# JihyongOh/DeMFI

Hardware: AMD Instinct MI355X
Metric: interpolated frames/sec @720p x8 MFI (N_tst=3) (higher is better)
Workload: dtype f16; 1 GPU; DeMFI-Net_rb N_tst=3, x8 MFI, 720x1280 (padded 736x1280), fp16, clip-parallel windows, random-init weights; uint8 frames host->HBM->host inside the timed region (PNG codec excluded), 8 distinct windows; graph=True, parallelism=clip1, n_ctx=7, n_trunk=3

## Files before the change

### demfi_amd/csrc/conv_wstream.hip

```cpp
#include "conv_common.h"

namespace {

#ifndef DEMFI_WS3_DEPTH
#define DEMFI_WS3_DEPTH 9
#endif
#ifndef DEMFI_WS_NW
#define DEMFI_WS_NW 4
#endif
template <int KS, int NW, int NCH = 2, int TH_ = 16> struct WsCfg {
    static constexpr int TH = TH_;
    static constexpr int RPW = TH / (NW / NCH);
    static constexpr int BL = KS + RPW - 1;
    static constexpr int LH = TH + KS - 1;
    static constexpr int LL = KS == 7 ? ((TW + KS - 1 + 7) & ~7) : TW + KS - 1;
    static constexpr int NI = (LH * LL + 15) / 16;
    static constexpr int UNIT_BYTES = NI * 1024;
    static constexpr int LDS_BYTES = 2 * UNIT_BYTES;
    static constexpr int NG = 2 * KS;
    static constexpr int NSTEP = NG * KS;
    static constexpr int DEPTH = NW == 8 ? KS : (KS == 7 ? 2 * KS : DEMFI_WS3_DEPTH);
    static constexpr int NIW = (NI + NW - 1) / NW;
    static constexpr int DMA_EVERY = KS == 7 ? 6 : 1;
    static constexpr int DMA_PER = KS == 7 ? 1 : 3;
    static constexpr bool PIECE_STRIDES = KS != 7;
    static_assert(LDS_BYTES <= 160 * 1024, "two units must fit LDS");
    static_assert((NIW + DMA_PER - 1) / DMA_PER * DMA_EVERY + DEPTH <= NSTEP, "the unit's DMA must be older than the last A fragment consumed in the unit");
    static_assert(NSTEP % DEPTH == 0, "static ring indices");
};

template <int KS, int NW, int NCH = 2, int TH_ = 16>
__global__ __launch_bounds__(64 * NW, 1) void conv_wstream_c64_kernel(const demfi_conv* __restrict__ d)
{
    using C = WsCfg<KS, NW, NCH, TH_>;
    constexpr int WS_TH = C::TH;
    constexpr int RPW = C::RPW;
    extern __shared__ __attribute__((aligned(16))) char smem[];
    const int tid = threadIdx.x;
    const int lane = tid & 63;
    const int wave = __builtin_amdgcn_readfirstlane(tid >> 6);
    const int hi = lane >> 5, lx = lane & 31;
    const int cs = NCH == 2 ? (wave & 1) : 0, rh = NCH == 2 ? (wave >> 1) : wave;
    const int H = d->H, W = d->W;
    const int tiles_x = (W + TW - 1) / TW, tiles_y = (H + WS_TH - 1) / WS_TH, tiles_img = tiles_x * tiles_y;
    const int total = tiles_img * d->batch;
    int t_first, t_end, t_step;
    {
        const int G = gridDim.x;
        if ((G & 7) == 0 && total >= G) {
            const int xcd = blockIdx.x & 7, idx = blockIdx.x >> 3;
            const int q = (total + 7) >> 3, lo = xcd * q;
            t_first = lo + idx;
            t_end = min(lo + q, total);
            t_step = G >> 3;
        } else {
            t_first = blockIdx.x;
            t_end = total;
            t_step = G;
        }
    }
    if (t_first >= t_end) return;
    const int upt = d->n_chunks;
    const int n_units = ((t_end - t_first + t_step - 1) / t_step) * upt;

    const demfi_piece& p0 = d->pieces[d->chunks[0].first_piece];
    const int64_t sxb = p0.v.sx * 2, syb = p0.v.sy * 2, sbb = p0.v.sb * 2;
    const char* const zeros = (const char*)d->zero_page;
    const uint4* const wbase = (const uint4*)d->wpack;

    int doff[C::NIW], dlc[C::NIW];
#pragma unroll
    for (int j = 0; j < C::NIW; ++j) {
        const int rec = min((wave + NW * j) * 16 + (lane >> 2), C::LH * C::LL - 1);
        const int l = rec / C::LL, c = rec - l * C::LL;
        doff[j] = C::PIECE_STRIDES ? (((lane & 3) ^ ((c >> 2) & 3)) << 4) : (int)(l * syb + c * sxb) + (((lane & 3) ^ ((c >> 2) & 3)) << 4);
        dlc[j] = l | (c << 8);
    }
    int boff[C::NG];
#pragma unroll
    for (int g = 0; g < C::NG; ++g) {
        const int col = lx + (g >> 1);
        boff[g] = (rh * RPW * C::LL + col) * 64 + ((((g & 1) * 2 + hi) ^ ((col >> 2) & 3)) << 4);
    }

    struct Unit { const char* src; const char* w; int iy0, ix0; bool interior; int sx, sy; };
    const unsigned lane16 = lane * 16;
    auto unit_info = [&](int u) {
        Unit r;
        const int k = u / upt, cu = u - k * upt;
        const int it = t_first + k * t_step;
        const int bimg = it / tiles_img, rem = it - bimg * tiles_img;
        const int ty = rem / tiles_x, tx = rem - ty * tiles_x;
        r.iy0 = ty * WS_TH - KS / 2;
        r.ix0 = tx * TW - KS / 2;
        const demfi_piece& pc = d->pieces[d->chunks[cu].first_piece];
        r.sx = C::PIECE_STRIDES ? (int)(pc.v.sx * 2) : (int)sxb;
        r.sy = C::PIECE_STRIDES ? (int)(pc.v.sy * 2) : (int)syb;
        r.src = (const char*)pc.v.ptr + bimg * (C::PIECE_STRIDES ? pc.v.sb * 2 : sbb) + (int64_t)r.iy0 * r.sy + (int64_t)r.ix0 * r.sx;
        r.w = (const char*)(wbase + d->chunks[cu].w_off + cs * 64);
        r.interior = r.iy0 >= 0 && r.iy0 + C::LH <= H && r.ix0 >= 0 && r.ix0 + C::LL <= W;
        return r;
    };
    auto dma_one = [&](auto J, const Unit& un, char* buf) {
        constexpr int j = decltype(J)::value;
        const int i = wave + NW * j;
        if (i >= C::NI) return;
        const char* g = un.src + doff[j];
        if constexpr (C::PIECE_STRIDES) g += (dlc[j] & 255) * un.sy + (dlc[j] >> 8) * un.sx;
        if (!un.interior) {
            const int iy = un.iy0 + (dlc[j] & 255), ix = un.ix0 + (dlc[j] >> 8);
            if (!(iy >= 0 && iy < H && ix >= 0 && ix < W)) g = zeros;
        }
        const unsigned la = (unsigned)(uintptr_t)(__attribute__((address_space(3))) char*)(buf + i * 1024);
#if defined(__HIP_DEVICE_COMPILE__)
        unsigned m0_save;
        asm volatile("s_mov_b32 %0, m0\n\ts_mov_b32 m0, %2\n\ts_nop 0\n\tglobal_load_lds_dwordx4 %1, off\n\ts_mov_b32 m0, %0"
                     : "=&s"(m0_save) : "v"(g), "s"(la) : "memory");
#endif
    };
    auto a_load = [&](const Unit& un, int t) {
        const int g = t / KS, ky = t - g * KS, kx = g >> 1, ksl = g & 1;
        return __builtin_bit_cast(uint4, *gcp<u4_t>(un.w + (unsigned)((((ky * KS + kx) * 2 + ksl) * NCH) * 1024 + lane16)));
    };

    const demfi_seg& sg = d->segs[d->sub_seg[0]];
    half_t* const dstp = (half_t*)sg.dst.ptr;
    const int act = sg.act;
    const int ch0 = d->oct_ch[0];
    f4_t bq[4];
#pragma unroll
    for (int qd = 0; qd < 4; ++qd) bq[qd] = *gcp<f4_t>(d->bias + cs * 32 + qd * 8 + hi * 4);

    f16x_t acc[RPW];
#pragma unroll
    for (int p = 0; p < RPW; ++p) {
#pragma unroll
        for (int i = 0; i < 16; ++i) acc[p][i] = 0.0f;
    }
    uint4 A[C::DEPTH];
    Unit cur = unit_info(0);
    static_for<0, C::NIW>([&](auto J) { dma_one(J, cur, smem); });
    static_for<0, C::DEPTH>([&](auto T) { A[decltype(T)::value] = a_load(cur, decltype(T)::value); });
    asm volatile("s_waitcnt vmcnt(%0)" ::"n"(C::DEPTH) : "memory");
    asm volatile("s_barrier" ::: "memory");

    for (int u = 0; u < n_units; ++u) {
        const bool has_next = u + 1 < n_units;
        TRACE_STAMP(wave, u / upt, u % upt);
        const Unit nxt = unit_info(has_next ? u + 1 : 0);
        const char* const tb = smem + (u & 1) * C::UNIT_BYTES;
        char* const nb = smem + ((u + 1) & 1) * C::UNIT_BYTES;
        uint4 B[2][C::BL];
#pragma unroll
        for (int r = 0; r < RPW; ++r) B[0][r] = *(const uint4*)(tb + boff[0] + r * (C::LL * 64));
        __builtin_amdgcn_sched_barrier(0);
        static_for<0, C::NSTEP>([&](auto T_) {
            constexpr int t = decltype(T_)::value;
            constexpr int g = t / KS, ky = t % KS, gb = g & 1;
            const uint4 a = A[t % C::DEPTH];
            if constexpr (ky + RPW < C::BL) B[gb][ky + RPW] = *(const uint4*)(tb + boff[g] + (ky + RPW) * (C::LL * 64));
            if constexpr (g + 1 < C::NG) {
                if constexpr (ky < RPW) B[gb ^ 1][ky] = *(const uint4*)(tb + boff[g + 1] + ky * (C::LL * 64));
                if constexpr (ky == KS - 1) {
#pragma unroll
                    for (int r = KS; r < RPW; ++r) B[gb ^ 1][r] = *(const uint4*)(tb + boff[g + 1] + r * (C::LL * 64));
                }
            }
            if constexpr (t + C::DEPTH < C::NSTEP) A[t % C::DEPTH] = a_load(cur, t + C::DEPTH);
            else                                   A[t % C::DEPTH] = a_load(nxt, t + C::DEPTH - C::NSTEP);
            if constexpr (KS == 7) {
                if constexpr (t % C::DMA_EVERY == 2 && t / C::DMA_EVERY < C::NIW) {
                    if (has_next) dma_one(std::integral_constant<int, t / C::DMA_EVERY>{}, nxt, nb);
                }
            } else {
                if (has_next) {
                    static_for<0, C::DMA_PER>([&](auto Q) {
                        constexpr int j = t * C::DMA_PER + decltype(Q)::value;
                        if constexpr (j < C::NIW) dma_one(std::integral_constant<int, j>{}, nxt, nb);
                    });
                }
            }
#pragma unroll
            for (int p = 0; p < RPW; ++p) Mma<half_t>::run(acc[p], a, B[gb][ky + p]);
            __builtin_amdgcn_sched_barrier(0);
        });
        asm volatile("s_waitcnt vmcnt(%0)" ::"n"(C::DEPTH) : "memory");
        const int k = u / upt;
        if (u - k * upt == upt - 1) {
            const int it = t_first + k * t_step;
            const int bimg = it / tiles_img, rem = it - bimg * tiles_img;
            const int ty = rem / tiles_x, tx = rem - ty * tiles_x;
            const int ox = tx * TW + lx;
#pragma unroll
            for (int p = 0; p < RPW; ++p) {
                const int oy = ty * WS_TH + rh * RPW + p;
#pragma unroll
                for (int m2 = 0; m2 < 2; ++m2) {
                    float v[8];
#pragma unroll
                    for (int j = 0; j < 4; ++j) {
                        v[j] = acc[p][(2 * m2) * 4 + j] + bq[2 * m2][j];
                        v[4 + j] = acc[p][(2 * m2 + 1) * 4 + j] + bq[2 * m2 + 1][j];
                    }
                    apply_act_n<8>(v, act);
                    if (oy < H && ox < W)
                        store8<half_t>(dstp + bimg * sg.dst.sb + oy * sg.dst.sy + ox * sg.dst.sx + ch0 + cs * 32 + m2 * 16 + hi * 8, v);
                }
#pragma unroll
                for (int i = 0; i < 16; ++i) acc[p][i] = 0.0f;
            }
        }
        asm volatile("s_barrier" ::: "memory");
        cur = nxt;
    }
}

static bool wstream_eligible(const demfi_conv* h, int ks = 7, int nch = 2)
{
    if (h->dtype != DEMFI_F16 || h->stride != 1 || h->kh != ks || h->kw != ks || h->pad_y != ks / 2 || h->pad_x != ks / 2) return false;
    if (h->inH != h->H || h->inW != h->W || !h->zero_page || h->rec_bytes != 64) return false;
    if (h->n_chunks < (ks == 7 ? 1 : 2) || h->cout_pad != 32 * nch || h->nco != nch) return false;
    const demfi_piece& p0 = h->pieces[h->chunks[0].first_piece];
    for (int c = 0; c < h->n_chunks; ++c) {
        const demfi_chunk& ch = h->chunks[c];
        if (ch.n_pieces != 1 || ch.nks != 2) return false;
        const demfi_piece& p = h->pieces[ch.first_piece];
        if (!p.fat || p.nch != 32 || p.up_shift || !p.v.ptr || p.v.sc != 1 || p.v.is_f32) return false;
        if (ks == 7 && (p.v.sx != p0.v.sx || p.v.sy != p0.v.sy || p.v.sb != p0.v.sb)) return false;
        if (p.v.sy < 0 || p.v.sx < 0 || p.v.sy >= (int64_t)1 << 31 || p.v.sx >= (int64_t)1 << 31) return false;
        if (p.v.sy * 2 * 40 + p.v.sx * 2 * 48 >= (int64_t)1 << 31) return false;
    }
    const int sgi = h->sub_seg[0];
    if (sgi < 0 || (nch == 2 && (h->sub_seg[1] != sgi || h->oct_ch[4] != h->oct_ch[0] + 32))) return false;
    for (int o = 0; o < 4 * nch; ++o)
        if (h->oct_seg[o] != sgi || h->oct_n[o] != 8 || h->oct_ch[o] != h->oct_ch[0] + 8 * o) return false;
    const demfi_seg& sg = h->segs[sgi];
    if (sg.mode != DEMFI_MODE_STORE || sg.scale != 1 || sg.dy || sg.dx || sg.res.ptr || !sg.dst.ptr || sg.dst.is_f32 || sg.dst.sc != 1) return false;
    return true;
}

static int launch_wstream3(const demfi_conv* h, const demfi_conv* dev, hipStream_t st)
{
    DEMFI_LDS_ATTR((conv_wstream_c64_kernel<3, 4, 1, 32>));
    const int total = ((h->W + TW - 1) / TW) * ((h->H + 31) / 32) * h->batch;
    const int grid = total >= 256 ? 256 : total;
    constexpr size_t lds = WsCfg<3, 4, 1, 32>::LDS_BYTES;
    hipLaunchKernelGGL((conv_wstream_c64_kernel<3, 4, 1, 32>), dim3(grid), dim3(256), lds, st, dev);
    DEMFI_HIP_CHECK(hipGetLastError());
    return DEMFI_OK;
}

static int launch_wstream(const demfi_conv* h, const demfi_conv* dev, hipStream_t st)
{
    DEMFI_LDS_ATTR((conv_wstream_c64_kernel<7, DEMFI_WS_NW>));
    const int total = ((h->W + TW - 1) / TW) * ((h->H + 15) / 16) * h->batch;
    const int grid = total >= 256 ? 256 : total;
    constexpr size_t lds = WsCfg<7, DEMFI_WS_NW>::LDS_BYTES;
    hipLaunchKernelGGL((conv_wstream_c64_kernel<7, DEMFI_WS_NW>), dim3(grid), dim3(64 * DEMFI_WS_NW), lds, st, dev);
    DEMFI_HIP_CHECK(hipGetLastError());
    return DEMFI_OK;
}


}

int demfi_wstream_trace_collect(unsigned long long* acc) { return TRACE_DRAIN(acc, true); }

bool demfi_wstream_eligible(const demfi_conv* h, int ks, int nch) { return wstream_eligible(h, ks, nch); }
int demfi_wstream_launch(const demfi_conv* h, const demfi_conv* dev, hipStream_t st) { return launch_wstream(h, dev, st); }
int demfi_wstream3_launch(const demfi_conv* h, const demfi_conv* dev, hipStream_t st) { return launch_wstream3(h, dev, st); }
```

### demfi_amd/csrc/gru.hip

```cpp
#include "kernel_kit.h"
#include <cstdlib>

namespace {

constexpr int G_LS = 32 * 128;
constexpr int G_NH = 4;
constexpr int G_NTHREADS = 256 + 64 * G_NH;
#ifndef DEMFI_GRU_DEPTH
#define DEMFI_GRU_DEPTH 4
#endif
constexpr int G_DEPTH = DEMFI_GRU_DEPTH;
constexpr int G_NSTEP = 20;
static_assert(G_NSTEP % G_DEPTH == 0, "static ring indices");
enum { GM_R = 1, GM_ZQS = 2 };
template <int MODE> struct GCfg;
template <> struct GCfg<GM_R>   { static constexpr int TL = 16, WL = 20, NPIECE = 2, LDS = 2 * 20 * G_LS; };
template <> struct GCfg<GM_ZQS> { static constexpr int TL = 8, WL = 12, NPIECE = 3, LDS = 3 * 12 * G_LS + 512; };
static_assert(GCfg<GM_R>::LDS <= 160 * 1024 && GCfg<GM_ZQS>::LDS <= 160 * 1024, "LDS budget");
constexpr int ZS_D = 8;
constexpr int ZS_NA = 80;
static_assert(ZS_NA % ZS_D == 0, "static ring indices");

DEMFI_TRACE_BUFFER(32, 8, 24, 10)

// ... 4 lines not shown
    asm("v_fma_mix_f32 %0, -%1, %2, %3 op_sel_hi:[1,0,0]" : "=v"(d) : "v"(h), "v"(b), "v"(c));
#endif
    return d;
}
__device__ __forceinline__ float g_nfma_hi(float b, unsigned h, float c)
{
    float d = 0.0f;
#if defined(__HIP_DEVICE_COMPILE__)
    asm("v_fma_mix_f32 %0, -%1, %2, %3 op_sel:[1,0,0] op_sel_hi:[1,0,0]" : "=v"(d) : "v"(h), "v"(b), "v"(c));
#endif
    return d;
}

__device__ __forceinline__ float g_sub16_lo(unsigned q, unsigned h)
{
    float d = 0.0f;
#if defined(__HIP_DEVICE_COMPILE__)
    asm("v_fma_mix_f32 %0, %1, -1.0, %2 op_sel_hi:[1,0,1]" : "=v"(d) : "v"(h), "v"(q));
#endif
    return d;
}
__device__ __forceinline__ float g_sub16_hi(unsigned q, unsigned h)
{
    float d = 0.0f;
#if defined(__HIP_DEVICE_COMPILE__)
    asm("v_fma_mix_f32 %0, %1, -1.0, %2 op_sel:[1,0,1] op_sel_hi:[1,0,1]" : "=v"(d) : "v"(h), "v"(q));
#endif
    return d;
}
__device__ __forceinline__ void g_fma16_lo(unsigned& pk, float a, float b, unsigned c)
{
#if defined(__HIP_DEVICE_COMPILE__)
    asm("v_fma_mixlo_f16 %0, %1, %2, %3 op_sel_hi:[0,0,1]" : "+v"(pk) : "v"(a), "v"(b), "v"(c));
#endif
}
__device__ __forceinline__ void g_fma16_hi(unsigned& pk, float a, float b, unsigned c)
{
#if defined(__HIP_DEVICE_COMPILE__)
    asm("v_fma_mixhi_f16 %0, %1, %2, %3 op_sel:[0,0,1] op_sel_hi:[0,0,1]" : "+v"(pk) : "v"(a), "v"(b), "v"(c));
#endif
}

struct GPiece { const char* ptr; int64_t sl, sp, sb; };
struct GArgs {
    GPiece h, rh, x;
    char* dst; int64_t d_sl, d_sp, d_sb;
    const char* w0[2];
    const char* w1[2];
    const float* b0; const float* b1;
    const char* zeros;
    int Llen, Plen, batch, n_pt, n_ls;
};

template <int MODE>
__global__ __launch_bounds__(G_NTHREADS, 1) void gru_sep5_kernel(const GArgs a)
{
    using Cfg = GCfg<MODE>;
    constexpr int TL = Cfg::TL, WL = Cfg::WL, PIECE = WL * G_LS;
    constexpr int NI = WL * 4, NIW = NI / G_NH;
    static_assert(NIW == WL, "helper dw owns pixels 8 dw .. 8 dw + 7 of every line");
    extern __shared__ __attribute__((aligned(16))) char smem[];
    const int tid = threadIdx.x;
    const int lane = tid & 63;
    const int wave = __builtin_amdgcn_readfirstlane(tid >> 6);
    const int per_img = a.n_pt * a.n_ls;
    const int total = per_img * a.batch;
    int it0, it1;
    XCD_ITEM_RUN(total, it0, it1);
    if (it0 >= it1) return;
    auto pos_of = [&](int it, int& img, int& P0, int& L0) {
        img = it / per_img;
        const int rem = it - img * per_img;
        const int pt = rem / a.n_ls;
        P0 = pt * 32;
        L0 = (rem - pt * a.n_ls) * TL;
    };
    char* const S0 = smem;
    char* const S1 = smem + PIECE;
    char* const S2 = smem + 2 * PIECE;

    if constexpr (MODE == GM_ZQS) {
        if (tid < 128) ((float*)(smem + 3 * PIECE))[tid] = tid < 64 ? a.b0[tid] : a.b1[tid - 64];
        asm volatile("s_waitcnt lgkmcnt(0)" ::: "memory");
    }
    if (wave >= 4) {
        const int dw = wave - 4;
        __builtin_assume(dw >= 0 && dw < G_NH);
        const int px = dw * 8 + (lane >> 3);
        const unsigned slot16 = (unsigned)(((lane & 7) ^ ((px >> 1) & 7)) << 4);
        auto issue_piece = [&](const GPiece& pc, char* lds, int img, int P0, int L0, bool carry) {
            const char* base = pc.ptr + (int64_t)img * pc.sb + (int64_t)(L0 - 2) * pc.sl + (int64_t)P0 * pc.sp;
            const unsigned voff = (unsigned)(px * pc.sp) + slot16;
            const bool pok = P0 + px < a.Plen;
            u4_t halo[4];
            if (carry) {
#pragma unroll
                for (int j = 0; j < 4; ++j) halo[j] = *(const u4_t*)(lds + (4 * (TL + j) + dw) * 1024 + lane * 16);
                asm volatile("s_waitcnt lgkmcnt(0)" ::: "memory");
            }
            if (L0 - 2 >= 0 && L0 - 2 + WL <= a.Llen && P0 + 32 <= a.Plen) {
#pragma unroll
                for (int k = 0; k < NIW; ++k) {
                    if (k < 4 && carry) continue;
                    const char* lb = base + (int64_t)k * pc.sl;
                    lb = (const char*)(((uint64_t)(unsigned)__builtin_amdgcn_readfirstlane((int)((uint64_t)lb >> 32)) << 32) |
                                       (uint64_t)(unsigned)__builtin_amdgcn_readfirstlane((int)(uint64_t)lb));
                    unsigned v = voff;
                    asm volatile("" : "+v"(v));
                    __builtin_amdgcn_global_load_lds((const DEMFI_GLOBAL void*)(lb + v),
// ... 160 lines not shown
                constexpr int n0 = NB + t * PER, n1 = n0 + PER - 1;
                const uint4 av0 = A[n0 % ZS_D];
                const uint4 av1 = A[n1 % ZS_D];
                if constexpr (tap < 4) B[4 + tap] = *(const uint4*)(tb + (4 + tap) * G_LS + boff(std::integral_constant<int, ks>{}));
                constexpr bool LA0 = n0 + ZS_D < ZS_NA, LA1 = DUAL && n1 + ZS_D < ZS_NA;
                if constexpr (LA0) A[n0 % ZS_D] = a_loadn(std::integral_constant<int, LA0 ? n0 + ZS_D : 0>{});
                if constexpr (LA1) A[n1 % ZS_D] = a_loadn(std::integral_constant<int, LA1 ? n1 + ZS_D : 0>{});
                constexpr bool NXT = tap == 4 && (ks < 3 || HASNEXT);
                const f16x_t zero = {};
                static_for<0, 4>([&](auto P) {
                    constexpr int p = decltype(P)::value;
                    if constexpr (WHICH != 1) {
                        if constexpr (t == 0 && NB != 40) Mma<half_t>::initc(accz[p], av0, B[tap + p], zero);
                        else Mma<half_t>::run(accz[p], av0, B[tap + p]);
                    }
                    if constexpr (WHICH != 0) {
                        if constexpr (t == 0 && NB != 40) Mma<half_t>::initc(accq[p], av1, B[tap + p], zero);
                        else Mma<half_t>::run(accq[p], av1, B[tap + p]);
                    }
                    if constexpr (NXT) B[p] = *(const uint4*)((ks < 3 ? tb : tbn) + p * G_LS + boff(std::integral_constant<int, (ks + 1) & 3>{}));
                });
                __builtin_amdgcn_sched_group_barrier(0x008, 1, 0);
                if constexpr (tap < 4 || NXT) __builtin_amdgcn_sched_group_barrier(0x100, 1, 0);
                __builtin_amdgcn_sched_group_barrier(0x008, 1, 0);
                if constexpr (LA0) __builtin_amdgcn_sched_group_barrier(0x020, 1, 0);
                if constexpr (NXT) __builtin_amdgcn_sched_group_barrier(0x100, 1, 0);
                __builtin_amdgcn_sched_group_barrier(0x008, 1, 0);
                if constexpr (LA1) __builtin_amdgcn_sched_group_barrier(0x020, 1, 0);
                if constexpr (NXT) __builtin_amdgcn_sched_group_barrier(0x100, 1, 0);
                __builtin_amdgcn_sched_group_barrier(0x008, 1, 0);
                if constexpr (NXT) __builtin_amdgcn_sched_group_barrier(0x100, 1, 0);
                if constexpr (DUAL) __builtin_amdgcn_sched_group_barrier(0x008, 4, 0);
                __builtin_amdgcn_sched_barrier(0);
            });
        };
        constexpr float KS_SIG = -1.4426950408889634f, KS_TANH = 2.8853900817779268f;
        typedef float f2_t __attribute__((ext_vector_type(2)));
        const char* const tbH = S0 + lh * 4 * G_LS;
        const char* const tbR = S1 + lh * 4 * G_LS;
        const char* const tbX = S2 + lh * 4 * G_LS;
        const float* const SB = (const float*)(smem + 3 * PIECE);
        int it = it0;
        [[maybe_unused]] int trk = 0;
        prime();
        TRACE_STAMP(wave, trk, 0);
        asm volatile("s_barrier" ::: "memory");
        for (;;) {
            int img, P0, L0;
            pos_of(it, img, P0, L0);
            TRACE_STAMP(wave, trk, 1);
            b_init(tbH);
            __builtin_amdgcn_sched_barrier(0);
            phase(tbH, tbR, std::integral_constant<int, 0>{}, std::integral_constant<int, 0>{}, std::true_type{});
            phase(tbR, tbR, std::integral_constant<int, 20>{}, std::integral_constant<int, 1>{}, std::false_type{});
            TRACE_STAMP(wave, trk, 2);
            asm volatile("s_barrier" ::: "memory");
            TRACE_STAMP(wave, trk, 3);
            b_init(tbX);
            __builtin_amdgcn_sched_barrier(0);
            phase(tbX, tbX, std::integral_constant<int, 40>{}, std::integral_constant<int, 2>{}, std::false_type{});
#if defined(__HIP_DEVICE_COMPILE__)
            asm volatile("" ::"v"(accz[0]), "v"(accz[1]), "v"(accz[2]), "v"(accz[3]), "v"(accq[0]), "v"(accq[1]), "v"(accq[2]), "v"(accq[3]));
#endif
            TRACE_STAMP(wave, trk, 4);
            asm volatile("s_barrier" ::: "memory");
            TRACE_STAMP(wave, trk, 5);
            const char* hb = a.h.ptr + (int64_t)img * a.h.sb + (int64_t)min(P0 + lx, a.Plen - 1) * a.h.sp + (cs * 32 + hi * 8) * 2;
            u4_t hreg[4][2];
#pragma unroll
            for (int p = 0; p < 4; ++p) {
                const char* hp = hb + (int64_t)min(L0 + lh * 4 + p, a.Llen - 1) * a.h.sl;
                hreg[p][0] = *gcp<u4_t>(hp);
                hreg[p][1] = *gcp<u4_t>(hp + 32);
            }
            __builtin_amdgcn_sched_barrier(0);
            {
                f2_t bz[8], bq[8];
#pragma unroll
                for (int g = 0; g < 4; ++g) {
                    const f4_t vz = *(const f4_t*)(SB + cs * 32 + g * 8 + hi * 4);
                    const f4_t vq = *(const f4_t*)(SB + 64 + cs * 32 + g * 8 + hi * 4);
                    bz[2 * g] = f2_t{vz[0], vz[1]} * KS_SIG;  bz[2 * g + 1] = f2_t{vz[2], vz[3]} * KS_SIG;
                    bq[2 * g] = f2_t{vq[0], vq[1]} * KS_TANH; bq[2 * g + 1] = f2_t{vq[2], vq[3]} * KS_TANH;
                }
                static_for<0, 4>([&](auto P) {
                    constexpr int p = decltype(P)::value;
#pragma unroll
                    for (int i = 0; i < 8; ++i) {
                        f2_t ez = f2_t{accz[p][2 * i], accz[p][2 * i + 1]} * KS_SIG + bz[i];
                        f2_t eq = f2_t{accq[p][2 * i], accq[p][2 * i + 1]} * KS_TANH + bq[i];
                        eq = f2_t{__builtin_fminf(eq.x, 60.0f), __builtin_fminf(eq.y, 60.0f)};
                        const f2_t av = f2_t{__builtin_amdgcn_exp2f(ez.x), __builtin_amdgcn_exp2f(ez.y)} + 1.0f;
                        const f2_t bv = f2_t{__builtin_amdgcn_exp2f(eq.x), __builtin_amdgcn_exp2f(eq.y)};
                        const f2_t den = (bv + 1.0f) * av;
                        accz[p][2 * i] = __builtin_amdgcn_rcpf(den.x);
                        accz[p][2 * i + 1] = __builtin_amdgcn_rcpf(den.y);
                        accq[p][2 * i] = bv.x;
                        accq[p][2 * i + 1] = bv.y;
                    }
                });
#if defined(__HIP_DEVICE_COMPILE__)
                asm volatile("" ::"v"(accz[0]), "v"(accz[1]), "v"(accz[2]), "v"(accz[3]), "v"(accq[0]), "v"(accq[1]), "v"(accq[2]), "v"(accq[3]));
#endif
                __builtin_amdgcn_sched_barrier(0);
                TRACE_STAMP(wave, trk, 6);
                static_for<0, 4>([&](auto P) {
                    constexpr int p = decltype(P)::value;
#pragma unroll
                    for (int m2 = 0; m2 < 2; ++m2) {
                        const u4_t rr = hreg[p][m2];
                        u4_t o = {0u, 0u, 0u, 0u};
#pragma unroll
                        for (int d = 0; d < 4; ++d) {
                            const int i0 = 8 * m2 + 2 * d;
                            const f2_t bv = f2_t{accq[p][i0], accq[p][i0 + 1]};
                            const f2_t bp = bv + 1.0f, bm = bv - 1.0f;
                            const float nlo = g_nfma_lo(bp.x, rr[d], bm.x);
                            const float nhi = g_nfma_hi(bp.y, rr[d], bm.y);
                            unsigned pk = 0u;
                            g_fma16_lo(pk, nlo, accz[p][i0], rr[d]);
                            g_fma16_hi(pk, nhi, accz[p][i0 + 1], rr[d]);
                            o[d] = pk;
                        }
                        *(u4_t*)(S2 + (lh * 4 + p) * G_LS + soff[m2]) = o;
                    }
                });
// ... 138 lines not shown
                const h8_t r = __builtin_bit_cast(h8_t, *(const u4_t*)(t1 + (2 + p) * G_LS + soff[m2]));
                h8_t o;
#pragma unroll
                for (int j = 0; j < 2; ++j) {
                    o[2 * j] = (half_t)__builtin_fmaf(sg[4 * m2 + j].x, (float)r[2 * j], 0.0f);
                    o[2 * j + 1] = (half_t)__builtin_fmaf(sg[4 * m2 + j].y, (float)r[2 * j + 1], 0.0f);
                    o[4 + 2 * j] = (half_t)__builtin_fmaf(sg[4 * m2 + 2 + j].x, (float)r[4 + 2 * j], 0.0f);
                    o[4 + 2 * j + 1] = (half_t)__builtin_fmaf(sg[4 * m2 + 2 + j].y, (float)r[4 + 2 * j + 1], 0.0f);
                }
                if (pok && l < a.Llen) *gp<u4_t>(ob + (int64_t)l * a.d_sl + m2 * 32) = __builtin_bit_cast(u4_t, o);
            }
        });
        TRACE_STAMP(wave, trk, 5);
        asm volatile("s_barrier" ::: "memory");
        ++trk;
        ++it;
        if (it >= it1) break;
    }
}

bool g_layer_ok(const demfi_conv* h)
{
    if (h->dtype != DEMFI_F16 || h->stride != 1 || !h->zero_page || !h->wpack || !h->bias || !h->cout_perm) return false;
    if (!((h->kh == 1 && h->kw == 5) || (h->kh == 5 && h->kw == 1))) return false;
    if (h->pad_y != h->kh / 2 || h->pad_x != h->kw / 2 || h->inH != h->H || h->inW != h->W) return false;
    if (h->n_chunks != 2 || h->cout_pad != 64 || h->nco != 2 || h->n_segs < 1) return false;
    for (int c = 0; c < 2; ++c) {
        const demfi_chunk& ch = h->chunks[c];
        if (ch.n_pieces != 1 || ch.nks != 4) return false;
        const demfi_piece& p = h->pieces[ch.first_piece];
        if (!p.fat || p.nch != 64 || p.up_shift || !p.v.ptr || p.v.sc != 1 || p.v.is_f32) return false;
        if (p.v.sy < 0 || p.v.sx < 0 || p.v.sy >= (int64_t)1 << 31 || p.v.sx >= (int64_t)1 << 31) return false;
        if (p.v.sy * 2 * 24 + p.v.sx * 2 * 40 >= (int64_t)1 << 31) return false;
    }
    const int sgi = h->sub_seg[0];
    if (sgi < 0 || h->sub_seg[1] != sgi) return false;
    for (int o = 0; o < 8; ++o)
        if (h->oct_seg[o] != sgi || h->oct_n[o] != 8 || h->oct_ch[o] != h->oct_ch[0] + 8 * o) return false;
    const demfi_seg& sg = h->segs[sgi];
    if (sg.scale != 1 || sg.dy || sg.dx || !sg.dst.ptr || sg.dst.is_f32 || sg.dst.sc != 1) return false;
    if (h->pack.ptr || h->u8_sink) return false;
    return true;
}
bool g_same_view(const demfi_view& a, const demfi_view& b)
{
    return a.ptr == b.ptr && a.sx == b.sx && a.sy == b.sy && a.sb == b.sb && a.sc == b.sc && a.is_f32 == b.is_f32;
}
GPiece g_piece(const demfi_view& v, bool tr)
{
    return GPiece{(const char*)v.ptr, (tr ? v.sy : v.sx) * 2, (tr ? v.sx : v.sy) * 2, v.sb * 2};
}
const char* g_wchunk(const demfi_conv* h, int c) { return (const char*)h->wpack + h->chunks[c].w_off * 16; }

template <int MODE>
int g_launch(GArgs& a, const demfi_conv* h, const demfi_seg& out, void* stream)
{
    const bool tr = h->kh == 5;
    a.dst = (char*)out.dst.ptr + (int64_t)h->oct_ch[0] * 2;
    a.d_sl = (tr ? out.dst.sy : out.dst.sx) * 2; a.d_sp = (tr ? out.dst.sx : out.dst.sy) * 2; a.d_sb = out.dst.sb * 2;
    a.zeros = (const char*)h->zero_page;
    a.Llen = tr ? h->H : h->W; a.Plen = tr ? h->W : h->H; a.batch = h->batch;
    a.n_pt = (a.Plen + 31) / 32;
    a.n_ls = (a.Llen + GCfg<MODE>::TL - 1) / GCfg<MODE>::TL;
    const int64_t total = (int64_t)a.n_pt * a.n_ls * a.batch;
    if (total <= 0 || total >= (int64_t)1 << 30) return demfi_set_error(DEMFI_ERR_ARG, "demfi_gru: empty or oversized launch");
    if (a.d_sl < 0 || a.d_sp < 0 || a.d_sl >= (int64_t)1 << 31 || a.d_sp >= (int64_t)1 << 31 || a.d_sl * 24 + a.d_sp * 40 >= (int64_t)1 << 31) return demfi_set_error(DEMFI_ERR_ARG, "demfi_gru: destination strides exceed 32-bit lane offsets");
    DEMFI_LDS_ATTR(gru_sep5_kernel<MODE>);
    const int grid = total >= 256 ? 256 : (int)total;
    hipLaunchKernelGGL(gru_sep5_kernel<MODE>, dim3(grid), dim3(G_NTHREADS), GCfg<MODE>::LDS, (hipStream_t)stream, a);
    DEMFI_HIP_CHECK(hipGetLastError());
    return DEMFI_OK;
}

}

extern "C" int demfi_gru_r_eligible(const demfi_conv* hr)
{
    if (!hr || !g_layer_ok(hr)) return 0;
    const demfi_seg& sg = hr->segs[hr->sub_seg[0]];
    if (sg.mode != DEMFI_MODE_MUL || !sg.res.ptr) return 0;
    const demfi_view& h = hr->pieces[hr->chunks[0].first_piece].v;
    demfi_view res = sg.res;
    res.ptr = (char*)res.ptr + (int64_t)hr->oct_ch[0] * 2;
    if (!g_same_view(res, h)) return 0;
    if (sg.dst.ptr == h.ptr) return 0;
    return 1;
}

extern "C" int demfi_gru_r(const demfi_conv* hr, void* stream)
{
    if (!demfi_gru_r_eligible(hr))
        return demfi_set_error(DEMFI_ERR_ARG, "demfi_gru_r: not the reset-gate layer of a SepConvGRU half-step (1x5 / 5x1 fp16, [h, x] -> 64, MUL epilogue with res == h)");
    const bool tr = hr->kh == 5;
    GArgs a = {};
    a.h = g_piece(hr->pieces[hr->chunks[0].first_piece].v, tr);
    a.x = g_piece(hr->pieces[hr->chunks[1].first_piece].v, tr);
    a.rh = a.h;
    a.w0[0] = g_wchunk(hr, 0); a.w0[1] = g_wchunk(hr, 1);
    a.w1[0] = a.w0[0]; a.w1[1] = a.w0[1];
    a.b0 = a.b1 = hr->bias;
    return g_launch<GM_R>(a, hr, hr->segs[hr->sub_seg[0]], stream);
}

extern "C" int demfi_gru_zq_eligible(const demfi_conv* hz, const demfi_conv* hq)
{
    if (!hz || !hq || !g_layer_ok(hz) || !g_layer_ok(hq)) return 0;
    if (hz->kh != hq->kh || hz->kw != hq->kw || hz->H != hq->H || hz->W != hq->W || hz->batch != hq->batch) return 0;
    const demfi_seg& sz = hz->segs[hz->sub_seg[0]];
    const demfi_seg& sq = hq->segs[hq->sub_seg[0]];
    if (sz.mode != DEMFI_MODE_STORE || sz.act != DEMFI_ACT_SIGMOID || sz.res.ptr) return 0;
    if (sq.mode != DEMFI_MODE_GRU || !sq.res.ptr || !sq.aux.ptr) return 0;
    const demfi_view& h = hz->pieces[hz->chunks[0].first_piece].v;
    const demfi_view& xz = hz->pieces[hz->chunks[1].first_piece].v;
    const demfi_view& xq = hq->pieces[hq->chunks[1].first_piece].v;
    if (!g_same_view(xz, xq)) return 0;
    demfi_view res = sq.res, aux = sq.aux, zd = sz.dst;
    res.ptr = (char*)res.ptr + (int64_t)hq->oct_ch[0] * 2;
    aux.ptr = (char*)aux.ptr + (int64_t)hq->oct_ch[0] * 2;
    zd.ptr = (char*)zd.ptr + (int64_t)hz->oct_ch[0] * 2;
    if (!g_same_view(res, h) || !g_same_view(aux, zd)) return 0;
    if (sq.dst.ptr == h.ptr) return 0;
    return 1;
}

extern "C" int demfi_gru_zq(const demfi_conv* hz, const demfi_conv* hq, void* stream)
{
    if (!demfi_gru_zq_eligible(hz, hq))
        return demfi_set_error(DEMFI_ERR_ARG, "demfi_gru_zq: not the (update gate, candidate) pair of a SepConvGRU half-step (1x5 / 5x1 fp16, [h, x] -> 64 "
                                              "sigmoid and [r*h, x] -> 64 with the GRU epilogue on the same h, x, z)");
    const bool tr = hz->kh == 5;
    GArgs a = {};
    a.h = g_piece(hz->pieces[hz->chunks[0].first_piece].v, tr);
    a.x = g_piece(hz->pieces[hz->chunks[1].first_piece].v, tr);
    a.rh = g_piece(hq->pieces[hq->chunks[0].first_piece].v, tr);
    a.w0[0] = g_wchunk(hz, 0); a.w0[1] = g_wchunk(hz, 1);
    a.w1[0] = g_wchunk(hq, 0); a.w1[1] = g_wchunk(hq, 1);
    a.b0 = hz->bias; a.b1 = hq->bias;
    return g_launch<GM_ZQS>(a, hq, hq->segs[hq->sub_seg[0]], stream);
}

#ifdef DEMFI_TRACE
extern "C" int demfi_gru_trace_dump(unsigned long long* out, int64_t n)
{
    if (n != TR_N) return demfi_set_error(DEMFI_ERR_ARG, "demfi_gru_trace_dump: expected %lld entries", (long long)TR_N);
    DEMFI_HIP_CHECK(hipDeviceSynchronize());
    return TRACE_DRAIN(out, false);
}
#endif
```

### demfi_amd/csrc/kernel_kit.h

```cpp
#pragma once
#include "common.h"
#include <type_traits>
#ifdef DEMFI_TRACE
#include <vector>
#endif

namespace {

template <int I, int N, typename F>
__device__ __forceinline__ void static_for(F&& f)
{
    if constexpr (I < N) {
        f(std::integral_constant<int, I>{});
        static_for<I + 1, N>(f);
    }
}

template <typename T> struct Mma;

template <> struct Mma<half_t> {
    static __device__ __forceinline__ void run(f16x_t& acc, const uint4& a, const uint4& b)
    {
        acc = __builtin_amdgcn_mfma_f32_32x32x16_f16(__builtin_bit_cast(h8_t, a), __builtin_bit_cast(h8_t, b),
                                                     acc, 0, 0, 0);
    }
    static __device__ __forceinline__ void initc(f16x_t& acc, const uint4& a, const uint4& b, const f16x_t& c)
    {
        acc = __builtin_amdgcn_mfma_f32_32x32x16_f16(__builtin_bit_cast(h8_t, a), __builtin_bit_cast(h8_t, b), c, 0, 0, 0);
    }
    static __device__ __forceinline__ void init(f16x_t& acc, const uint4& a, const uint4& b)
    {
        const f16x_t z = {0.f, 0.f, 0.f, 0.f, 0.f, 0.f, 0.f, 0.f, 0.f, 0.f, 0.f, 0.f, 0.f, 0.f, 0.f, 0.f};
        acc = __builtin_amdgcn_mfma_f32_32x32x16_f16(__builtin_bit_cast(h8_t, a), __builtin_bit_cast(h8_t, b), z, 0, 0, 0);
    }
};
template <> struct Mma<float> {
    static __device__ __forceinline__ void run(f16x_t& acc, const uint4& a, const uint4& b)
    {
        f4_t fa = __builtin_bit_cast(f4_t, a), fb = __builtin_bit_cast(f4_t, b);
        acc = __builtin_amdgcn_mfma_f32_32x32x2f32(fa[0], fb[0], acc, 0, 0, 0);
        acc = __builtin_amdgcn_mfma_f32_32x32x2f32(fa[1], fb[1], acc, 0, 0, 0);
        acc = __builtin_amdgcn_mfma_f32_32x32x2f32(fa[2], fb[2], acc, 0, 0, 0);
        acc = __builtin_amdgcn_mfma_f32_32x32x2f32(fa[3], fb[3], acc, 0, 0, 0);
    }
};

__device__ __forceinline__ float res_mix_lo(unsigned a, float c)
{
    float d = 0.0f;
#if defined(__HIP_DEVICE_COMPILE__)
    asm("v_fma_mix_f32 %0, %1, 1.0, %2 op_sel_hi:[1,0,0]" : "=v"(d) : "v"(a), "v"(c));
#endif
    return d;
}
__device__ __forceinline__ float res_mix_hi(unsigned a, float c)
{
    float d = 0.0f;
#if defined(__HIP_DEVICE_COMPILE__)
    asm("v_fma_mix_f32 %0, %1, 1.0, %2 op_sel:[1,0,0] op_sel_hi:[1,0,0]" : "=v"(d) : "v"(a), "v"(c));
#endif
    return d;
}
__device__ __forceinline__ float sub_mix_lo(float c, unsigned a)
{
    float d = 0.0f;
#if defined(__HIP_DEVICE_COMPILE__)
    asm("v_fma_mix_f32 %0, %1, -1.0, %2 op_sel_hi:[1,0,0]" : "=v"(d) : "v"(a), "v"(c));
#endif
    return d;
}
__device__ __forceinline__ float sub_mix_hi(float c, unsigned a)
{
    float d = 0.0f;
#if defined(__HIP_DEVICE_COMPILE__)
    asm("v_fma_mix_f32 %0, %1, -1.0, %2 op_sel:[1,0,0] op_sel_hi:[1,0,0]" : "=v"(d) : "v"(a), "v"(c));
#endif
    return d;
}

#define XCD_ITEM_RUN(total_, it0_, it1_)                                                                             \
    {                                                                                                                 \
        const int G = gridDim.x;                                                                                      \
        if ((G & 7) == 0 && (total_) >= G) {                                                                          \
            const int xcd = blockIdx.x & 7, idx = blockIdx.x >> 3, nw = G >> 3;                                       \
            const int q = (total_) >> 3, r = (total_) & 7;                                                            \
            const int lo = xcd * q + min(xcd, r), n = q + (xcd < r ? 1 : 0);                                          \
// ... 54 lines not shown
```

Measured before the change: 102.7 frames/s.

## Add 16x16x32 MFMA variant of wstream conv and LDS-sourced GRU hidden state

Adds an optional 16x16x32 MFMA instantiation of the 7x7 weight-streaming conv kernel. It reorganizes A/B fragment loads, accumulators, the DMA offset computation and the epilogue for that shape, and is selected by an env var that defaults to the existing 32x32 form. Separately, the GRU ZQS kernel now reads the hidden state from the LDS window it has already staged, instead of issuing global loads after the barriers. That GRU path is enabled by default and is meant to remove global-memory latency from the critical path, at the cost of extra live registers across a phase.

Measured after the change: 103.1 frames/s, median of 6. No clear change (+0.4%).

```diff
diff --git a/demfi_amd/csrc/conv_wstream.hip b/demfi_amd/csrc/conv_wstream.hip
--- a/demfi_amd/csrc/conv_wstream.hip
+++ b/demfi_amd/csrc/conv_wstream.hip
@@ -8,7 +8,10 @@
 #ifndef DEMFI_WS_NW
 #define DEMFI_WS_NW 4
 #endif
-template <int KS, int NW, int NCH = 2, int TH_ = 16> struct WsCfg {
+template <int KS, int NW, int NCH = 2, int TH_ = 16, int MSHAPE = 32> struct WsCfg {
+    static_assert(MSHAPE == 32 || (MSHAPE == 16 && KS == 7 && NCH == 2), "the 16x16x32 form exists for the 7x7 / 64-cout instantiation");
+    static constexpr bool M16 = MSHAPE == 16;
+    static constexpr int NA = M16 ? 2 : 1;
     static constexpr int TH = TH_;
     static constexpr int RPW = TH / (NW / NCH);
     static constexpr int BL = KS + RPW - 1;
@@ -17,11 +20,11 @@
     static constexpr int NI = (LH * LL + 15) / 16;
     static constexpr int UNIT_BYTES = NI * 1024;
     static constexpr int LDS_BYTES = 2 * UNIT_BYTES;
-    static constexpr int NG = 2 * KS;
+    static constexpr int NG = M16 ? KS : 2 * KS;
     static constexpr int NSTEP = NG * KS;
-    static constexpr int DEPTH = NW == 8 ? KS : (KS == 7 ? 2 * KS : DEMFI_WS3_DEPTH);
+    static constexpr int DEPTH = NW == 8 || M16 ? KS : (KS == 7 ? 2 * KS : DEMFI_WS3_DEPTH);
     static constexpr int NIW = (NI + NW - 1) / NW;
-    static constexpr int DMA_EVERY = KS == 7 ? 6 : 1;
+    static constexpr int DMA_EVERY = KS == 7 ? (M16 ? 3 : 6) : 1;
     static constexpr int DMA_PER = KS == 7 ? 1 : 3;
     static constexpr bool PIECE_STRIDES = KS != 7;
     static_assert(LDS_BYTES <= 160 * 1024, "two units must fit LDS");
@@ -29,10 +32,10 @@
     static_assert(NSTEP % DEPTH == 0, "static ring indices");
 };
 
-template <int KS, int NW, int NCH = 2, int TH_ = 16>
+template <int KS, int NW, int NCH = 2, int TH_ = 16, int MSHAPE = 32>
 __global__ __launch_bounds__(64 * NW, 1) void conv_wstream_c64_kernel(const demfi_conv* __restrict__ d)
 {
-    using C = WsCfg<KS, NW, NCH, TH_>;
+    using C = WsCfg<KS, NW, NCH, TH_, MSHAPE>;
     constexpr int WS_TH = C::TH;
     constexpr int RPW = C::RPW;
     extern __shared__ __attribute__((aligned(16))) char smem[];
@@ -68,19 +71,24 @@
     const char* const zeros = (const char*)d->zero_page;
     const uint4* const wbase = (const uint4*)d->wpack;
 
-    int doff[C::NIW], dlc[C::NIW];
-#pragma unroll
-    for (int j = 0; j < C::NIW; ++j) {
-        const int rec = min((wave + NW * j) * 16 + (lane >> 2), C::LH * C::LL - 1);
+    auto dma_rec = [&](int j, int ln, int& off, int& lc) {
+        const int rec = min((wave + NW * j) * 16 + (ln >> 2), C::LH * C::LL - 1);
         const int l = rec / C::LL, c = rec - l * C::LL;
-        doff[j] = C::PIECE_STRIDES ? (((lane & 3) ^ ((c >> 2) & 3)) << 4) : (int)(l * syb + c * sxb) + (((lane & 3) ^ ((c >> 2) & 3)) << 4);
-        dlc[j] = l | (c << 8);
-    }
+        off = C::PIECE_STRIDES ? (((ln & 3) ^ ((c >> 2) & 3)) << 4) : (int)(l * syb + c * sxb) + (((ln & 3) ^ ((c >> 2) & 3)) << 4);
+        lc = l | (c << 8);
+    };
+    int doff[C::M16 ? 1 : C::NIW], dlc[C::M16 ? 1 : C::NIW];
+    if constexpr (!C::M16) {
+#pragma unroll
+        for (int j = 0; j < C::NIW; ++j) dma_rec(j, lane, doff[j], dlc[j]);
+    }
+    const int n16 = lane & 15, g16 = lane >> 4;
     int boff[C::NG];
 #pragma unroll
     for (int g = 0; g < C::NG; ++g) {
-        const int col = lx + (g >> 1);
-        boff[g] = (rh * RPW * C::LL + col) * 64 + ((((g & 1) * 2 + hi) ^ ((col >> 2) & 3)) << 4);
+        const int col = C::M16 ? n16 + g : lx + (g >> 1);
+        const int slot = C::M16 ? g16 : (g & 1) * 2 + hi;
+        boff[g] = (rh * RPW * C::LL + col) * 64 + ((slot ^ ((col >> 2) & 3)) << 4);
     }
 
     struct Unit { const char* src; const char* w; int iy0, ix0; bool interior; int sx, sy; };
@@ -105,10 +113,19 @@
         constexpr int j = decltype(J)::value;
         const int i = wave + NW * j;
         if (i >= C::NI) return;
-        const char* g = un.src + doff[j];
-        if constexpr (C::PIECE_STRIDES) g += (dlc[j] & 255) * un.sy + (dlc[j] >> 8) * un.sx;
+        int off, lc;
+        if constexpr (C::M16) {
+            int ln = lane;
+            asm volatile("" : "+v"(ln));
+            dma_rec(j, ln, off, lc);
+        } else {
+            off = doff[j];
+            lc = dlc[j];
+        }
+        const char* g = un.src + off;
+        if constexpr (C::PIECE_STRIDES) g += (lc & 255) * un.sy + (lc >> 8) * un.sx;
         if (!un.interior) {
-            const int iy = un.iy0 + (dlc[j] & 255), ix = un.ix0 + (dlc[j] >> 8);
+            const int iy = un.iy0 + (lc & 255), ix = un.ix0 + (lc >> 8);
             if (!(iy >= 0 && iy < H && ix >= 0 && ix < W)) g = zeros;
         }
         const unsigned la = (unsigned)(uintptr_t)(__attribute__((address_space(3))) char*)(buf + i * 1024);
@@ -122,26 +139,54 @@
         const int g = t / KS, ky = t - g * KS, kx = g >> 1, ksl = g & 1;
         return __builtin_bit_cast(uint4, *gcp<u4_t>(un.w + (unsigned)((((ky * KS + kx) * 2 + ksl) * NCH) * 1024 + lane16)));
     };
+    const unsigned alane16 = (unsigned)((g16 >> 1) * NCH * 1024 + ((g16 & 1) * 32 + n16) * 16);
+    auto a_load16 = [&](const Unit& un, int t, int cb) {
+        const int kx = t / KS, ky = t - kx * KS;
+        return __builtin_bit_cast(uint4, *gcp<u4_t>(un.w + (unsigned)(((ky * KS + kx) * 2 * NCH) * 1024 + cb * 256 + alane16)));
+    };
 
     const demfi_seg& sg = d->segs[d->sub_seg[0]];
     half_t* const dstp = (half_t*)sg.dst.ptr;
     const int act = sg.act;
     const int ch0 = d->oct_ch[0];
-    f4_t bq[4];
-#pragma unroll
-    for (int qd = 0; qd < 4; ++qd) bq[qd] = *gcp<f4_t>(d->bias + cs * 32 + qd * 8 + hi * 4);
-
-    f16x_t acc[RPW];
-#pragma unroll
-    for (int p = 0; p < RPW; ++p) {
-#pragma unroll
-        for (int i = 0; i < 16; ++i) acc[p][i] = 0.0f;
-    }
-    uint4 A[C::DEPTH];
+    constexpr int NPB = C::M16 ? 2 : 1;
+    f4_t bq[C::M16 ? 2 : 4];
+    if constexpr (C::M16) {
+#pragma unroll
+        for (int cb = 0; cb < 2; ++cb) bq[cb] = *gcp<f4_t>(d->bias + cs * 32 + cb * 16 + g16 * 4);
+    } else {
+#pragma unroll
+        for (int qd = 0; qd < 4; ++qd) bq[qd] = *gcp<f4_t>(d->bias + cs * 32 + qd * 8 + hi * 4);
+    }
+
+    f16x_t acc[C::M16 ? 1 : RPW];
+    f4_t acc4[C::M16 ? RPW : 1][2][2];
+    if constexpr (C::M16) {
+#pragma unroll
+        for (int p = 0; p < RPW; ++p)
+#pragma unroll
+            for (int q = 0; q < 4; ++q) acc4[p][q >> 1][q & 1] = f4_t{0.0f, 0.0f, 0.0f, 0.0f};
+    } else {
+#pragma unroll
+        for (int p = 0; p < RPW; ++p) {
+#pragma unroll
+            for (int i = 0; i < 16; ++i) acc[p][i] = 0.0f;
+        }
+    }
+    uint4 A[C::DEPTH][C::NA];
+    auto a_fill = [&](auto S, const Unit& un, int t) {
+        constexpr int sl = decltype(S)::value;
+        if constexpr (C::M16) {
+            A[sl][0] = a_load16(un, t, 0);
+            A[sl][1] = a_load16(un, t, 1);
+        } else {
+            A[sl][0] = a_load(un, t);
+        }
+    };
     Unit cur = unit_info(0);
     static_for<0, C::NIW>([&](auto J) { dma_one(J, cur, smem); });
-    static_for<0, C::DEPTH>([&](auto T) { A[decltype(T)::value] = a_load(cur, decltype(T)::value); });
-    asm volatile("s_waitcnt vmcnt(%0)" ::"n"(C::DEPTH) : "memory");
+    static_for<0, C::DEPTH>([&](auto T) { a_fill(T, cur, decltype(T)::value); });
+    asm volatile("s_waitcnt vmcnt(%0)" ::"n"(C::DEPTH * C::NA) : "memory");
     asm volatile("s_barrier" ::: "memory");
 
     for (int u = 0; u < n_units; ++u) {
@@ -150,24 +195,30 @@
         const Unit nxt = unit_info(has_next ? u + 1 : 0);
         const char* const tb = smem + (u & 1) * C::UNIT_BYTES;
         char* const nb = smem + ((u + 1) & 1) * C::UNIT_BYTES;
-        uint4 B[2][C::BL];
-#pragma unroll
-        for (int r = 0; r < RPW; ++r) B[0][r] = *(const uint4*)(tb + boff[0] + r * (C::LL * 64));
+        uint4 B[2][C::BL][NPB];
+#pragma unroll
+        for (int r = 0; r < RPW; ++r)
+#pragma unroll
+            for (int pb = 0; pb < NPB; ++pb) B[0][r][pb] = *(const uint4*)(tb + boff[0] + pb * 1024 + r * (C::LL * 64));
         __builtin_amdgcn_sched_barrier(0);
         static_for<0, C::NSTEP>([&](auto T_) {
             constexpr int t = decltype(T_)::value;
             constexpr int g = t / KS, ky = t % KS, gb = g & 1;
-            const uint4 a = A[t % C::DEPTH];
-            if constexpr (ky + RPW < C::BL) B[gb][ky + RPW] = *(const uint4*)(tb + boff[g] + (ky + RPW) * (C::LL * 64));
-            if constexpr (g + 1 < C::NG) {
-                if constexpr (ky < RPW) B[gb ^ 1][ky] = *(const uint4*)(tb + boff[g + 1] + ky * (C::LL * 64));
-                if constexpr (ky == KS - 1) {
-#pragma unroll
-                    for (int r = KS; r < RPW; ++r) B[gb ^ 1][r] = *(const uint4*)(tb + boff[g + 1] + r * (C::LL * 64));
+            const uint4 a = A[t % C::DEPTH][0];
+            [[maybe_unused]] const uint4 a1 = A[t % C::DEPTH][C::NA - 1];
+#pragma unroll
+            for (int pb = 0; pb < NPB; ++pb) {
+                if constexpr (ky + RPW < C::BL) B[gb][ky + RPW][pb] = *(const uint4*)(tb + boff[g] + pb * 1024 + (ky + RPW) * (C::LL * 64));
+                if constexpr (g + 1 < C::NG) {
+                    if constexpr (ky < RPW) B[gb ^ 1][ky][pb] = *(const uint4*)(tb + boff[g + 1] + pb * 1024 + ky * (C::LL * 64));
+                    if constexpr (ky == KS - 1) {
+#pragma unroll
+                        for (int r = KS; r < RPW; ++r) B[gb ^ 1][r][pb] = *(const uint4*)(tb + boff[g + 1] + pb * 1024 + r * (C::LL * 64));
+                    }
                 }
             }
-            if constexpr (t + C::DEPTH < C::NSTEP) A[t % C::DEPTH] = a_load(cur, t + C::DEPTH);
-            else                                   A[t % C::DEPTH] = a_load(nxt, t + C::DEPTH - C::NSTEP);
+            if constexpr (t + C::DEPTH < C::NSTEP) a_fill(std::integral_constant<int, t % C::DEPTH>{}, cur, t + C::DEPTH);
+            else                                   a_fill(std::integral_constant<int, t % C::DEPTH>{}, nxt, t + C::DEPTH - C::NSTEP);
             if constexpr (KS == 7) {
                 if constexpr (t % C::DMA_EVERY == 2 && t / C::DMA_EVERY < C::NIW) {
                     if (has_next) dma_one(std::integral_constant<int, t / C::DMA_EVERY>{}, nxt, nb);
@@ -180,34 +231,66 @@
                     });
                 }
             }
-#pragma unroll
-            for (int p = 0; p < RPW; ++p) Mma<half_t>::run(acc[p], a, B[gb][ky + p]);
+            if constexpr (C::M16) {
+#pragma unroll
+                for (int p = 0; p < RPW; ++p) {
+                    Mma16::run(acc4[p][0][0], a, B[gb][ky + p][0]);
+                    Mma16::run(acc4[p][0][1], a, B[gb][ky + p][NPB - 1]);
+                    Mma16::run(acc4[p][1][0], a1, B[gb][ky + p][0]);
+                    Mma16::run(acc4[p][1][1], a1, B[gb][ky + p][NPB - 1]);
+                }
+            } else {
+#pragma unroll
+                for (int p = 0; p < RPW; ++p) Mma<half_t>::run(acc[p], a, B[gb][ky + p][0]);
+            }
             __builtin_amdgcn_sched_barrier(0);
         });
-        asm volatile("s_waitcnt vmcnt(%0)" ::"n"(C::DEPTH) : "memory");
+        asm volatile("s_waitcnt vmcnt(%0)" ::"n"(C::DEPTH * C::NA) : "memory");
         const int k = u / upt;
         if (u - k * upt == upt - 1) {
             const int it = t_first + k * t_step;
             const int bimg = it / tiles_img, rem = it - bimg * tiles_img;
             const int ty = rem / tiles_x, tx = rem - ty * tiles_x;
-            const int ox = tx * TW + lx;
-#pragma unroll
-            for (int p = 0; p < RPW; ++p) {
-                const int oy = ty * WS_TH + rh * RPW + p;
-#pragma unroll
-                for (int m2 = 0; m2 < 2; ++m2) {
-                    float v[8];
-#pragma unroll
-                    for (int j = 0; j < 4; ++j) {
-                        v[j] = acc[p][(2 * m2) * 4 + j] + bq[2 * m2][j];
-                        v[4 + j] = acc[p][(2 * m2 + 1) * 4 + j] + bq[2 * m2 + 1][j];
+            if constexpr (C::M16) {
+#pragma unroll
+                for (int p = 0; p < RPW; ++p) {
+                    const int oy = ty * WS_TH + rh * RPW + p;
+#pragma unroll
+                    for (int q = 0; q < 4; ++q) {
+                        const int cb = q >> 1, pb = q & 1;
+                        const int ox = tx * TW + pb * 16 + n16;
+                        float v[4];
+#pragma unroll
+                        for (int j = 0; j < 4; ++j) v[j] = acc4[p][cb][pb][j] + bq[cb][j];
+                        apply_act_n<4>(v, act);
+                        h4_t o;
+#pragma unroll
+                        for (int j = 0; j < 4; ++j) o[j] = (half_t)v[j];
+                        if (oy < H && ox < W)
+                            *gp<h4_t>(dstp + bimg * sg.dst.sb + oy * sg.dst.sy + ox * sg.dst.sx + ch0 + cs * 32 + cb * 16 + (g16 & 1) * 8 + (g16 >> 1) * 4) = o;
+                        acc4[p][cb][pb] = f4_t{0.0f, 0.0f, 0.0f, 0.0f};
                     }
-                    apply_act_n<8>(v, act);
-                    if (oy < H && ox < W)
-                        store8<half_t>(dstp + bimg * sg.dst.sb + oy * sg.dst.sy + ox * sg.dst.sx + ch0 + cs * 32 + m2 * 16 + hi * 8, v);
-                }
-#pragma unroll
-                for (int i = 0; i < 16; ++i) acc[p][i] = 0.0f;
+                }
+            } else {
+                const int ox = tx * TW + lx;
+#pragma unroll
+                for (int p = 0; p < RPW; ++p) {
+                    const int oy = ty * WS_TH + rh * RPW + p;
+#pragma unroll
+                    for (int m2 = 0; m2 < 2; ++m2) {
+                        float v[8];
+#pragma unroll
+                        for (int j = 0; j < 4; ++j) {
+                            v[j] = acc[p][(2 * m2) * 4 + j] + bq[2 * m2][j];
+                            v[4 + j] = acc[p][(2 * m2 + 1) * 4 + j] + bq[2 * m2 + 1][j];
+                        }
+                        apply_act_n<8>(v, act);
+                        if (oy < H && ox < W)
+                            store8<half_t>(dstp + bimg * sg.dst.sb + oy * sg.dst.sy + ox * sg.dst.sx + ch0 + cs * 32 + m2 * 16 + hi * 8, v);
+                    }
+#pragma unroll
+                    for (int i = 0; i < 16; ++i) acc[p][i] = 0.0f;
+                }
             }
         }
         asm volatile("s_barrier" ::: "memory");
@@ -250,15 +333,26 @@
     return DEMFI_OK;
 }
 
-static int launch_wstream(const demfi_conv* h, const demfi_conv* dev, hipStream_t st)
-{
-    DEMFI_LDS_ATTR((conv_wstream_c64_kernel<7, DEMFI_WS_NW>));
+template <int MSHAPE>
+static int launch_wstream_shape(const demfi_conv* h, const demfi_conv* dev, hipStream_t st)
+{
+    DEMFI_LDS_ATTR((conv_wstream_c64_kernel<7, DEMFI_WS_NW, 2, 16, MSHAPE>));
     const int total = ((h->W + TW - 1) / TW) * ((h->H + 15) / 16) * h->batch;
     const int grid = total >= 256 ? 256 : total;
-    constexpr size_t lds = WsCfg<7, DEMFI_WS_NW>::LDS_BYTES;
-    hipLaunchKernelGGL((conv_wstream_c64_kernel<7, DEMFI_WS_NW>), dim3(grid), dim3(64 * DEMFI_WS_NW), lds, st, dev);
+    constexpr size_t lds = WsCfg<7, DEMFI_WS_NW, 2, 16, MSHAPE>::LDS_BYTES;
+    hipLaunchKernelGGL((conv_wstream_c64_kernel<7, DEMFI_WS_NW, 2, 16, MSHAPE>), dim3(grid), dim3(64 * DEMFI_WS_NW), lds, st, dev);
     DEMFI_HIP_CHECK(hipGetLastError());
     return DEMFI_OK;
+}
+
+#ifndef DEMFI_WS_MFMA_DEFAULT
+#define DEMFI_WS_MFMA_DEFAULT 32
+#endif
+static int launch_wstream(const demfi_conv* h, const demfi_conv* dev, hipStream_t st)
+{
+    static const int shape = [] { const char* e = getenv("DEMFI_WS_MFMA"); const int v = e ? atoi(e) : 0; return v == 16 || v == 32 ? v : DEMFI_WS_MFMA_DEFAULT; }();
+    if (shape == 16) return launch_wstream_shape<16>(h, dev, st);
+    return launch_wstream_shape<32>(h, dev, st);
 }
 
 
diff --git a/demfi_amd/csrc/gru.hip b/demfi_amd/csrc/gru.hip
--- a/demfi_amd/csrc/gru.hip
+++ b/demfi_amd/csrc/gru.hip
@@ -80,9 +80,10 @@
     int Llen, Plen, batch, n_pt, n_ls;
 };
 
-template <int MODE>
+template <int MODE, bool HLDS = false>
 __global__ __launch_bounds__(G_NTHREADS, 1) void gru_sep5_kernel(const GArgs a)
 {
+    static_assert(MODE == GM_ZQS || !HLDS, "the R launch has always read h from its window");
     using Cfg = GCfg<MODE>;
     constexpr int TL = Cfg::TL, WL = Cfg::WL, PIECE = WL * G_LS;
     constexpr int NI = WL * 4, NIW = NI / G_NH;
@@ -349,7 +350,20 @@
             b_init(tbH);
             __builtin_amdgcn_sched_barrier(0);
             phase(tbH, tbR, std::integral_constant<int, 0>{}, std::integral_constant<int, 0>{}, std::true_type{});
+            u4_t hreg[4][2];
+            if constexpr (HLDS) {
+#if defined(__HIP_DEVICE_COMPILE__)
+                asm volatile("" ::"v"(accz[0]), "v"(accz[1]), "v"(accz[2]), "v"(accz[3]));
+#endif
+#pragma unroll
+                for (int p = 0; p < 4; ++p) {
+                    hreg[p][0] = *(const u4_t*)(tbH + (2 + p) * G_LS + soff[0]);
+                    hreg[p][1] = *(const u4_t*)(tbH + (2 + p) * G_LS + soff[1]);
+                }
+                __builtin_amdgcn_sched_barrier(0);
+            }
             phase(tbR, tbR, std::integral_constant<int, 20>{}, std::integral_constant<int, 1>{}, std::false_type{});
+            if constexpr (HLDS) asm volatile("s_waitcnt lgkmcnt(0)" ::: "memory");
             TRACE_STAMP(wave, trk, 2);
             asm volatile("s_barrier" ::: "memory");
             TRACE_STAMP(wave, trk, 3);
@@ -362,13 +376,14 @@
             TRACE_STAMP(wave, trk, 4);
             asm volatile("s_barrier" ::: "memory");
             TRACE_STAMP(wave, trk, 5);
-            const char* hb = a.h.ptr + (int64_t)img * a.h.sb + (int64_t)min(P0 + lx, a.Plen - 1) * a.h.sp + (cs * 32 + hi * 8) * 2;
-            u4_t hreg[4][2];
-#pragma unroll
-            for (int p = 0; p < 4; ++p) {
-                const char* hp = hb + (int64_t)min(L0 + lh * 4 + p, a.Llen - 1) * a.h.sl;
-                hreg[p][0] = *gcp<u4_t>(hp);
-                hreg[p][1] = *gcp<u4_t>(hp + 32);
+            if constexpr (!HLDS) {
+                const char* hb = a.h.ptr + (int64_t)img * a.h.sb + (int64_t)min(P0 + lx, a.Plen - 1) * a.h.sp + (cs * 32 + hi * 8) * 2;
+#pragma unroll
+                for (int p = 0; p < 4; ++p) {
+                    const char* hp = hb + (int64_t)min(L0 + lh * 4 + p, a.Llen - 1) * a.h.sl;
+                    hreg[p][0] = *gcp<u4_t>(hp);
+                    hreg[p][1] = *gcp<u4_t>(hp + 32);
+                }
             }
             __builtin_amdgcn_sched_barrier(0);
             {
@@ -613,7 +628,7 @@
 }
 const char* g_wchunk(const demfi_conv* h, int c) { return (const char*)h->wpack + h->chunks[c].w_off * 16; }
 
-template <int MODE>
+template <int MODE, bool HLDS = false>
 int g_launch(GArgs& a, const demfi_conv* h, const demfi_seg& out, void* stream)
 {
     const bool tr = h->kh == 5;
@@ -626,9 +641,9 @@
     const int64_t total = (int64_t)a.n_pt * a.n_ls * a.batch;
     if (total <= 0 || total >= (int64_t)1 << 30) return demfi_set_error(DEMFI_ERR_ARG, "demfi_gru: empty or oversized launch");
     if (a.d_sl < 0 || a.d_sp < 0 || a.d_sl >= (int64_t)1 << 31 || a.d_sp >= (int64_t)1 << 31 || a.d_sl * 24 + a.d_sp * 40 >= (int64_t)1 << 31) return demfi_set_error(DEMFI_ERR_ARG, "demfi_gru: destination strides exceed 32-bit lane offsets");
-    DEMFI_LDS_ATTR(gru_sep5_kernel<MODE>);
+    DEMFI_LDS_ATTR((gru_sep5_kernel<MODE, HLDS>));
     const int grid = total >= 256 ? 256 : (int)total;
-    hipLaunchKernelGGL(gru_sep5_kernel<MODE>, dim3(grid), dim3(G_NTHREADS), GCfg<MODE>::LDS, (hipStream_t)stream, a);
+    hipLaunchKernelGGL((gru_sep5_kernel<MODE, HLDS>), dim3(grid), dim3(G_NTHREADS), GCfg<MODE>::LDS, (hipStream_t)stream, a);
     DEMFI_HIP_CHECK(hipGetLastError());
     return DEMFI_OK;
 }
@@ -697,7 +712,9 @@
     a.w0[0] = g_wchunk(hz, 0); a.w0[1] = g_wchunk(hz, 1);
     a.w1[0] = g_wchunk(hq, 0); a.w1[1] = g_wchunk(hq, 1);
     a.b0 = hz->bias; a.b1 = hq->bias;
-    return g_launch<GM_ZQS>(a, hq, hq->segs[hq->sub_seg[0]], stream);
+    static const bool hlds = [] { const char* e = getenv("DEMFI_GRU_HLDS"); return !(e && atoi(e) == 0); }();
+    if (hlds) return g_launch<GM_ZQS, true>(a, hq, hq->segs[hq->sub_seg[0]], stream);
+    return g_launch<GM_ZQS, false>(a, hq, hq->segs[hq->sub_seg[0]], stream);
 }
 
 #ifdef DEMFI_TRACE
diff --git a/demfi_amd/csrc/kernel_kit.h b/demfi_amd/csrc/kernel_kit.h
--- a/demfi_amd/csrc/kernel_kit.h
+++ b/demfi_amd/csrc/kernel_kit.h
@@ -32,6 +32,12 @@
     {
         const f16x_t z = {0.f, 0.f, 0.f, 0.f, 0.f, 0.f, 0.f, 0.f, 0.f, 0.f, 0.f, 0.f, 0.f, 0.f, 0.f, 0.f};
         acc = __builtin_amdgcn_mfma_f32_32x32x16_f16(__builtin_bit_cast(h8_t, a), __builtin_bit_cast(h8_t, b), z, 0, 0, 0);
+    }
+};
+struct Mma16 {
+    static __device__ __forceinline__ void run(f4_t& acc, const uint4& a, const uint4& b)
+    {
+        acc = __builtin_amdgcn_mfma_f32_16x16x32_f16(__builtin_bit_cast(h8_t, a), __builtin_bit_cast(h8_t, b), acc, 0, 0, 0);
     }
 };
 template <> struct Mma<float> {
```
